# ALVI-Labs/frankenstein

Hardware: AMD Instinct MI355X
Metric: neural frames/sec (train fwd+bwd+AdamW, whole job) (higher is better)
Workload: dtype bf16; 1 GPU; brainformer-small (6L d=384 6x64 heads, N=6144 tokens) + 2-block perceiver, L1 head; fwd+bwd+clip+AdamW; per_gpu_batch=32, global_batch=32, frames_T=600, electrodes=256, parallelism=dp1, weights=random-init (seed 42)

## Files before the change

frankenstein_amd/csrc/elementwise.hip:

```cpp
#include "fk_common.h"

namespace {

template <typename T>
__global__ void rope_kernel(T* x, int64_t B, int64_t T_, int64_t ld, int rot_cols, int D, const float* table,
                            int64_t table_bs, int64_t pos_off, float sgn) {
  constexpr int N = VecIO<T>::N;
  const int cpr = rot_cols / N;
  const int64_t total = B * T_ * cpr;
  for (int64_t i = blockIdx.x * (int64_t)blockDim.x + threadIdx.x; i < total; i += (int64_t)gridDim.x * blockDim.x) {
    const int ch = (int)(i % cpr);
    const int64_t row = i / cpr, t = row % T_, b = row / T_;
    const int col = ch * N, d = col % D;
    T* px = x + row * ld + col;
    const float* tb = table + b * table_bs + ((pos_off + t) * (D / 2) + d / 2) * 2;
    float v[N], o[N];
    VecIO<T>::load(px, v);
#pragma unroll
    for (int j = 0; j < N / 2; ++j) {
      const float c = tb[2 * j], s = sgn * tb[2 * j + 1];
      o[2 * j] = v[2 * j] * c - v[2 * j + 1] * s;
      o[2 * j + 1] = v[2 * j] * s + v[2 * j + 1] * c;
    }
    VecIO<T>::store(px, o);
// ... 35 lines not shown
}
template <typename T>
__global__ void swiglu_bwd_kernel(const T* h13, const T* dg, T* dh13, int64_t rows, int H) {
  constexpr int N = VecIO<T>::N;
  const int cpr = H / N;
  const int64_t total = rows * cpr;
  for (int64_t i = blockIdx.x * (int64_t)blockDim.x + threadIdx.x; i < total; i += (int64_t)gridDim.x * blockDim.x) {
    const int64_t r = i / cpr;
    const int c = (int)(i % cpr) * N;
    float a[N], b[N], d[N], oa[N], ob[N];
    VecIO<T>::load(h13 + r * 2 * H + c, a);
    VecIO<T>::load(h13 + r * 2 * H + H + c, b);
    VecIO<T>::load(dg + r * H + c, d);
#pragma unroll
    for (int j = 0; j < N; ++j) {
      const float sg = sigmoidf_(a[j]);
      oa[j] = d[j] * b[j] * sg * (1.0f + a[j] * (1.0f - sg));
      ob[j] = d[j] * a[j] * sg;
    }
    VecIO<T>::store(dh13 + r * 2 * H + c, oa);
    VecIO<T>::store(dh13 + r * 2 * H + H + c, ob);
  }
}
template <typename T>
__global__ void gelu_fwd_kernel(const T* x, T* y, int64_t nvec) {
  constexpr int N = VecIO<T>::N;
  for (int64_t i = blockIdx.x * (int64_t)blockDim.x + threadIdx.x; i < nvec; i += (int64_t)gridDim.x * blockDim.x) {
    float a[N], o[N];
    VecIO<T>::load(x + i * N, a);
#pragma unroll
    for (int j = 0; j < N; ++j) o[j] = fk_gelu(a[j]);
    VecIO<T>::store(y + i * N, o);
  }
}
template <typename T>
__global__ void dropout_kernel(const T* x, const T* res, T* y, int64_t nvec, const unsigned* seed, unsigned site, unsigned thresh, float ks) {
  constexpr int N = VecIO<T>::N;
  const DropKey key = drop_key(seed, site, thresh);
  for (int64_t i = blockIdx.x * (int64_t)blockDim.x + threadIdx.x; i < nvec; i += (int64_t)gridDim.x * blockDim.x) {
    float a[N], o[N];
    VecIO<T>::load(x + i * N, a);
    if (res) VecIO<T>::load(res + i * N, o);
    const int64_t e0 = i * N;
    const unsigned row = drop_row(key, (unsigned)(e0 >> 32));
#pragma unroll
    for (int j = 0; j < N; ++j) {
      const float v = drop_keep(key, row, (unsigned)e0 + j) ? a[j] * ks : 0.0f;
      o[j] = res ? o[j] + v : v;
    }
    VecIO<T>::store(y + i * N, o);
  }
}
template <typename T>
__global__ void gelu_bwd_kernel(const T* x, const T* dy, T* dx, int64_t nvec) {
  constexpr int N = VecIO<T>::N;
  for (int64_t i = blockIdx.x * (int64_t)blockDim.x + threadIdx.x; i < nvec; i += (int64_t)gridDim.x * blockDim.x) {
    float a[N], d[N], o[N];
    VecIO<T>::load(x + i * N, a);
    VecIO<T>::load(dy + i * N, d);
#pragma unroll
    for (int j = 0; j < N; ++j) {
      const float cdf = 0.5f * (1.0f + erff(a[j] * 0.70710678118654752f));
      const float pdf = 0.3989422804014327f * __expf(-0.5f * a[j] * a[j]);
      o[j] = d[j] * (cdf + a[j] * pdf);
    }
    VecIO<T>::store(dx + i * N, o);
  }
}

template <typename T>
__global__ void cast_pack_kernel(const float* src, int64_t lds, T* dst, int64_t ldd, int rows, int cols, int transpose,
                                 int rblk, int rstride, int roff) {
  const int64_t total = (int64_t)rows * cols;
  for (int64_t i = blockIdx.x * (int64_t)blockDim.x + threadIdx.x; i < total; i += (int64_t)gridDim.x * blockDim.x) {
    int r, c;
    if (transpose) { r = (int)(i % rows); c = (int)(i / rows); }
    else { r = (int)(i / cols); c = (int)(i % cols); }
    const int rd = rblk > 0 ? (r / rblk) * rstride + (r % rblk) + roff : r;
    const float v = src[(int64_t)r * lds + c];
    if (transpose) dst[(int64_t)c * ldd + rd] = from_f32<T>(v);
    else dst[(int64_t)rd * ldd + c] = from_f32<T>(v);
  }
}
template <typename T>
__global__ __launch_bounds__(256) void cast_pack_multi_kernel(const fk_pack_job* jobs, int njobs, int64_t total_chunks) {
  __shared__ float tile[32][33];
  for (int64_t ch = blockIdx.x; ch < total_chunks; ch += gridDim.x) {
    int lo = 0, hi = njobs - 1;
    while (lo < hi) {
      const int mid = (lo + hi + 1) >> 1;
      if (jobs[mid].chunk_begin <= ch) lo = mid; else hi = mid - 1;
    }
    const fk_pack_job jb = jobs[lo];
    T* dst = (T*)jb.dst;
    const int64_t local = ch - jb.chunk_begin;
    if (!jb.transpose) {
      const int64_t total = (int64_t)jb.rows * jb.cols, base = local * 1024;
#pragma unroll
      for (int q = 0; q < 4; ++q) {
        const int64_t i = base + q * 256 + threadIdx.x;
        if (i >= total) break;
        const int r = (int)(i / jb.cols), c = (int)(i % jb.cols);
        const int rd = jb.rblk > 0 ? (r / jb.rblk) * jb.rstride + (r % jb.rblk) + jb.roff : r;
        dst[(int64_t)rd * jb.ldd + c] = from_f32<T>(jb.src[(int64_t)r * jb.lds + c]);
      }
    } else {
      const int tcols = (jb.cols + 31) / 32;
      const int r0 = (int)(local / tcols) * 32, c0 = (int)(local % tcols) * 32;
      const int tx = threadIdx.x & 31, ty = threadIdx.x >> 5;
      __syncthreads();
#pragma unroll
      for (int q = 0; q < 4; ++q) {
        const int r = r0 + ty + 8 * q, c = c0 + tx;
        tile[ty + 8 * q][tx] = (r < jb.rows && c < jb.cols) ? jb.src[(int64_t)r * jb.lds + c] : 0.0f;
      }
      __syncthreads();
#pragma unroll
      for (int q = 0; q < 4; ++q) {
        const int c = c0 + ty + 8 * q, r = r0 + tx;
        if (r < jb.rows && c < jb.cols) {
          const int rd = jb.rblk > 0 ? (r / jb.rblk) * jb.rstride + (r % jb.rblk) + jb.roff : r;
          dst[(int64_t)c * jb.ldd + rd] = from_f32<T>(tile[tx][ty + 8 * q]);
        }
      }
    }
  }
}
template <typename TS, typename TD>
__global__ void cast_kernel(const TS* src, TD* dst, int64_t n) {
  for (int64_t i = blockIdx.x * (int64_t)blockDim.x + threadIdx.x; i < n; i += (int64_t)gridDim.x * blockDim.x)
    dst[i] = from_f32<TD>(to_f32<TS>(src[i]));
}
template <typename T>
__global__ void add_kernel(const T* a, const T* b, T* y, int64_t n) {
  for (int64_t i = blockIdx.x * (int64_t)blockDim.x + threadIdx.x; i < n; i += (int64_t)gridDim.x * blockDim.x)
    y[i] = from_f32<T>(to_f32<T>(a[i]) + to_f32<T>(b[i]));
}
template <typename T>
__global__ void copy2d_kernel(const T* src, int64_t lds, T* dst, int64_t ldd, int64_t rows, int64_t cols) {
  const int64_t total = rows * cols;
  for (int64_t i = blockIdx.x * (int64_t)blockDim.x + threadIdx.x; i < total; i += (int64_t)gridDim.x * blockDim.x)
    dst[(i / cols) * ldd + (i % cols)] = src[(i / cols) * lds + (i % cols)];
}

__global__ void add2d_kernel(const float* src, int64_t lds, float* dst, int64_t ldd, int64_t rows, int64_t cols) {
  const int64_t total = rows * cols;
  for (int64_t i = blockIdx.x * (int64_t)blockDim.x + threadIdx.x; i < total; i += (int64_t)gridDim.x * blockDim.x)
    dst[(i / cols) * ldd + (i % cols)] += src[(i / cols) * lds + (i % cols)];
}

template <typename T>
__global__ void gpt_embed_kernel(const int64_t* idx, const T* prefix, const float* wte, const float* wpe, T* out, int B,
                                 int t_ctx, int t_words, int dim, int vocab) {
  const int t_full = t_ctx + t_words;
  const int64_t total = (int64_t)B * t_full * dim;
  for (int64_t i = blockIdx.x * (int64_t)blockDim.x + threadIdx.x; i < total; i += (int64_t)gridDim.x * blockDim.x) {
    const int c = (int)(i % dim);
    const int64_t row = i / dim;
    const int t = (int)(row % t_full), b = (int)(row / t_full);
    float v;
    if (t < t_ctx) v = to_f32<T>(prefix[((int64_t)b * t_ctx + t) * dim + c]);
    else {
      int64_t id = idx[(int64_t)b * t_words + (t - t_ctx)];
      id = id < 0 ? 0 : (id >= vocab ? vocab - 1 : id);
      v = wte[id * dim + c];
    }
    out[i] = from_f32<T>(v + wpe[(int64_t)t * dim + c]);
  }
}
template <typename T>
__global__ void embed_bwd_kernel(const int64_t* idx, const T* dout, int64_t ldo_rows_per_b, int t_ctx, int t_words,
                                 float* dtable, int B, int dim, int vocab) {
  const int64_t total = (int64_t)B * t_words * dim;
  for (int64_t i = blockIdx.x * (int64_t)blockDim.x + threadIdx.x; i < total; i += (int64_t)gridDim.x * blockDim.x) {
    const int c = (int)(i % dim);
    const int64_t r = i / dim;
    const int j = (int)(r % t_words), b = (int)(r / t_words);
    int64_t id = idx[r];
    id = id < 0 ? 0 : (id >= vocab ? vocab - 1 : id);
    const float g = to_f32<T>(dout[((int64_t)b * ldo_rows_per_b + t_ctx + j) * dim + c]);
    atomicAdd(dtable + id * dim + c, g);
  }
}

template <typename TS, typename TD>
__global__ void gather_rows_kernel(const TS* src, int64_t src_bs, const int64_t* idx, int64_t idx_mod, TD* dst, int B, int n,
                                   int W, int scatter, int64_t dst_bs) {
  const int64_t total = (int64_t)B * n * W;
  for (int64_t i = blockIdx.x * (int64_t)blockDim.x + threadIdx.x; i < total; i += (int64_t)gridDim.x * blockDim.x) {
    const int c = (int)(i % W);
    const int64_t r = i / W;
    const int b = (int)(r / n), k = (int)(r % n);
    int64_t j = idx[r];
    if (idx_mod > 0) j %= idx_mod;
    if (scatter) dst[(int64_t)b * dst_bs + j * W + c] = from_f32<TD>(to_f32<TS>(src[(int64_t)b * src_bs + (int64_t)k * W + c]));
    else dst[(int64_t)b * dst_bs + (int64_t)k * W + c] = from_f32<TD>(to_f32<TS>(src[(int64_t)b * src_bs + j * W + c]));
  }
}
template <typename TS, typename TD>
__global__ __launch_bounds__(256) void gather_rows_vec_kernel(const TS* src, int64_t src_bs, const int64_t* idx, int64_t idx_mod, TD* dst, int B, int n,
                                                              int W, int scatter, int64_t dst_bs) {
  const int cpr = W >> 3;
  const int lane = threadIdx.x & 63;
  const int rpw = cpr >= 64 ? 1 : 64 / cpr;
  const int sub = cpr >= 64 ? 0 : lane / cpr;
// ... 310 lines not shown
```

frankenstein_amd/csrc/fk_common.h:

```cpp
#pragma once
#include <hip/hip_runtime.h>
#include <stdint.h>

#include "../../include/franken_hip.h"

typedef __bf16 bf16_t;
typedef __bf16 bf16x8 __attribute__((ext_vector_type(8)));
typedef __bf16 bf16x4 __attribute__((ext_vector_type(4)));
typedef __bf16 bf16x2 __attribute__((ext_vector_type(2)));
typedef float f32x16 __attribute__((ext_vector_type(16)));
typedef float f32x4 __attribute__((ext_vector_type(4)));
typedef float f32x2 __attribute__((ext_vector_type(2)));
typedef short s16x4 __attribute__((ext_vector_type(4)));
typedef unsigned int u32x4 __attribute__((ext_vector_type(4)));

#define FK_DEV __device__ __forceinline__

int fk_set_error(int code, const char* fmt, ...);
#define FK_CHECK_ARG(cond, ...)                                   \
  do {                                                            \
    if (!(cond)) return fk_set_error(FK_EINVAL, __VA_ARGS__);     \
  } while (0)
#define FK_CHECK_LAUNCH(name)                                                         \
  do {                                                                                \
    hipError_t e__ = hipGetLastError();                                               \
    if (e__ != hipSuccess) return fk_set_error(FK_ELAUNCH, "%s: %s", name, hipGetErrorString(e__)); \
  } while (0)

#define FK_DT_CHECK(name) FK_CHECK_ARG(dtype == FK_F32 || dtype == FK_BF16, name ": bad dtype %d", dtype)

static inline int64_t fk_cdiv(int64_t a, int64_t b) { return (a + b - 1) / b; }

constexpr int FK_TPB = 256;
static inline unsigned fk_grid(int64_t work, int64_t cap) {
  int64_t b = fk_cdiv(work, FK_TPB);
  if (b > cap) b = cap;
  if (b < 1) b = 1;
  return (unsigned)b;
}

#define FK_BY_DTYPE(dtype, T, ...)                                \
  do {                                                            \
    if ((dtype) == FK_BF16) { using T = bf16_t; __VA_ARGS__; }    \
    else { using T = float; __VA_ARGS__; }                        \
  } while (0)
#define FK_BY_DTYPE2(dtype_a, TA, dtype_b, TB, ...) FK_BY_DTYPE(dtype_a, TA, FK_BY_DTYPE(dtype_b, TB, __VA_ARGS__))

template <auto Kernel, typename Args>
static inline void fk_launch_lds(dim3 grid, dim3 block, size_t lds, hipStream_t s, const Args& a) {
  static const bool once = hipFuncSetAttribute(reinterpret_cast<const void*>(Kernel), hipFuncAttributeMaxDynamicSharedMemorySize, (int)lds) == hipSuccess;
  (void)once;
  hipLaunchKernelGGL(Kernel, grid, block, lds, s, a);
}

template <typename T> FK_DEV float to_f32(T v);
template <> FK_DEV float to_f32<float>(float v) { return v; }
template <> FK_DEV float to_f32<bf16_t>(bf16_t v) { return (float)v; }
template <typename T> FK_DEV T from_f32(float v);
template <> FK_DEV float from_f32<float>(float v) { return v; }
template <> FK_DEV bf16_t from_f32<bf16_t>(float v) { return (bf16_t)v; }

template <typename T> struct Frag;
template <> struct Frag<bf16_t> { bf16x8 v; };
template <> struct Frag<float> { float v[8]; };

template <typename T> FK_DEV void frag_zero(Frag<T>& f);
template <> FK_DEV void frag_zero<bf16_t>(Frag<bf16_t>& f) {
#pragma unroll
  for (int e = 0; e < 8; ++e) f.v[e] = (bf16_t)0.0f;
}
template <> FK_DEV void frag_zero<float>(Frag<float>& f) {
#pragma unroll
  for (int e = 0; e < 8; ++e) f.v[e] = 0.0f;
}

template <typename T> FK_DEV void frag_set(Frag<T>& f, int e, float x);
template <> FK_DEV void frag_set<bf16_t>(Frag<bf16_t>& f, int e, float x) { f.v[e] = (bf16_t)x; }
template <> FK_DEV void frag_set<float>(Frag<float>& f, int e, float x) { f.v[e] = x; }

template <typename T> FK_DEV void mma32(f32x16& acc, const Frag<T>& a, const Frag<T>& b);
template <> FK_DEV void mma32<bf16_t>(f32x16& acc, const Frag<bf16_t>& a, const Frag<bf16_t>& b) {
  acc = __builtin_amdgcn_mfma_f32_32x32x16_bf16(a.v, b.v, acc, 0, 0, 0);
}
template <> FK_DEV void mma32<float>(f32x16& acc, const Frag<float>& a, const Frag<float>& b) {
#pragma unroll
// ... 4 lines not shown
FK_DEV int acc_row_of_slot(int s, int h, int e) { return 16 * s + 8 * (e >> 2) + 4 * h + (e & 3); }

template <typename T> FK_DEV void frag_from_acc(Frag<T>& f, const f32x16& x, int s) {
#pragma unroll
  for (int e = 0; e < 8; ++e) frag_set<T>(f, e, x[8 * s + e]);
}

template <typename T> FK_DEV void frag_load_contig(Frag<T>& f, const T* p);
template <> FK_DEV void frag_load_contig<bf16_t>(Frag<bf16_t>& f, const bf16_t* p) {
  f.v = *reinterpret_cast<const bf16x8*>(p);
}
template <> FK_DEV void frag_load_contig<float>(Frag<float>& f, const float* p) {
  f32x4 a = *reinterpret_cast<const f32x4*>(p);
  f32x4 b = *reinterpret_cast<const f32x4*>(p + 4);
#pragma unroll
  for (int e = 0; e < 4; ++e) { f.v[e] = a[e]; f.v[4 + e] = b[e]; }
}

FK_DEV bf16x4 lds_read_tr4(const bf16_t* p) {
  s16x4 r = __builtin_amdgcn_ds_read_tr16_b64_v4i16(
      (__attribute__((address_space(3))) s16x4*)(__attribute__((address_space(3))) void*)p);
  return __builtin_bit_cast(bf16x4, r);
}

FK_DEV float fk_gelu(float x) { return 0.5f * x * (1.0f + erff(x * 0.70710678118654752f)); }

template <int STOP = 1> FK_DEV float wave_sum(float v) {
#pragma unroll
  for (int o = 32; o >= STOP; o >>= 1) v += __shfl_xor(v, o, 64);
  return v;
}
template <int STOP = 1> FK_DEV float wave_max(float v) {
#pragma unroll
  for (int o = 32; o >= STOP; o >>= 1) v = fmaxf(v, __shfl_xor(v, o, 64));
  return v;
}

FK_DEV unsigned fk_mix32(unsigned x) {
  x ^= x >> 16; x *= 0x7feb352du; x ^= x >> 15; x *= 0x846ca68bu; x ^= x >> 16;
  return x;
}
struct DropKey { unsigned seed, salt, thresh; };
FK_DEV DropKey drop_key(const unsigned* seed_ptr, unsigned site, unsigned thresh) {
  return DropKey{seed_ptr[0], seed_ptr[1] * 0x85EBCA6Bu + site, thresh};
}
FK_DEV unsigned drop_row(const DropKey& k, unsigned hi) { return fk_mix32(fk_mix32(hi ^ k.seed) + k.salt); }
FK_DEV bool drop_keep(const DropKey& k, unsigned row, unsigned lo) { return fk_mix32(row ^ (lo * 0x9E3779B9u)) >= k.thresh; }

template <bool NT, typename V> FK_DEV void fk_st(V* q, const V& v) {
  if constexpr (NT) __builtin_nontemporal_store(v, q);
  else *q = v;
}

template <typename T, bool NT = false> struct VecIO;
template <bool NT> struct VecIO<bf16_t, NT> {
  static constexpr int N = 8;
  FK_DEV static void load(const bf16_t* p, float (&v)[8]) {
    bf16x8 a = *reinterpret_cast<const bf16x8*>(p);
#pragma unroll
    for (int i = 0; i < 8; ++i) v[i] = (float)a[i];
  }
  FK_DEV static void store(bf16_t* p, const float (&v)[8]) {
    bf16x8 a;
#pragma unroll
    for (int i = 0; i < 8; ++i) a[i] = (bf16_t)v[i];
    fk_st<NT>(reinterpret_cast<bf16x8*>(p), a);
  }
};
template <bool NT> struct VecIO<float, NT> {
  static constexpr int N = 4;
  FK_DEV static void load(const float* p, float (&v)[4]) {
    f32x4 a = *reinterpret_cast<const f32x4*>(p);
#pragma unroll
    for (int i = 0; i < 4; ++i) v[i] = a[i];
  }
  FK_DEV static void store(float* p, const float (&v)[4]) {
    f32x4 a;
#pragma unroll
    for (int i = 0; i < 4; ++i) a[i] = v[i];
    *reinterpret_cast<f32x4*>(p) = a;
  }
};

FK_DEV unsigned xcd_remap(unsigned bid, unsigned nwg) {
  const unsigned q = nwg >> 3, r = nwg & 7u, x = bid & 7u, i = bid >> 3;
  return (x < r ? x * (q + 1) : r * (q + 1) + (x - r) * q) + i;
}
```

frankenstein_amd/csrc/gemm.hip:

```cpp
#include <type_traits>

#include "fk_common.h"

namespace {

#ifndef FK_EPI_UNROLL
#define FK_EPI_UNROLL 1
#endif
#include "gemm_tile.h"

struct NtArgs {
  const void* A; const void* B; void* C;
  const void* bias; const void* res;
  int64_t lda, ldb, ldc, ldr, res_rows;
  int M, N, K, vec_epi;
  int mode;
  void* aux; int64_t ldaux;
  const float* rope_table; int64_t rope_bs; int rope_T, rope_off, rope_D, rope_cols;
  int rope_qcols; int64_t rope_qoff;
};

#ifndef FK_NT_STORES_GEMM
#define FK_NT_STORES_GEMM 1
#endif
// ... 1213 lines not shown
#endif
      __builtin_amdgcn_sched_barrier(0);
    }
  };
  using Yes = std::true_type;
  using No = std::false_type;
  using Vm0 = std::integral_constant<int, 0>;
  using Vm1 = std::integral_constant<int, PER>;
#pragma unroll
  for (int s = 0; s < TG_NS - 1; ++s)
    if (s < nk)
#pragma unroll
      for (int j = 0; j < PER; ++j) piece(s, j);
  if (nk > 0) {
    if (nk >= 3) vm_wait_barrier<2 * PER>(); else if (nk == 2) vm_wait_barrier<PER>(); else vm_wait_barrier<0>();
#pragma unroll
    for (int q = 0; q < NF; ++q) frag(f0, S0{}, q, 0);
#ifdef FK_TN_PROBE_HOIST
#pragma unroll
    for (int q = 0; q < NF; ++q) frag(f1, S1{}, q, 0);
#endif
    int kt = 0;
    for (; kt + TG_NS - 1 < nk; ++kt) step(Yes{}, Yes{}, Vm1{});
    if (kt + 2 < nk) { step(Yes{}, No{}, Vm1{}); ++kt; }
    if (kt + 1 < nk) step(Yes{}, No{}, Vm0{});
    step(No{}, No{}, Vm0{});
  }

  float* out = (p.nsplit > 1) ? p.ws + (int64_t)split * p.N1 * p.N2 : p.C;
  const int64_t ldo = (p.nsplit > 1) ? p.N2 : p.ldc;
  const bool accum = (p.nsplit == 1) && p.accumulate;
#pragma unroll
  for (int j = 0; j < NJ; ++j) {
    const int n = b0 + wn * WB + j * 32 + li;
#pragma unroll
    for (int i = 0; i < 3; ++i)
#pragma unroll
      for (int r = 0; r < 16; ++r) {
        const int m = a0 + wm * 96 + i * 32 + acc_row(r, lh);
        float* dst = out + (int64_t)m * ldo + n;
        *dst = accum ? (*dst + acc[i][j][r]) : acc[i][j][r];
      }
  }
}

template <bool IL>
__global__ __launch_bounds__(256) void reduce_slabs4_kernel(const float* ws, float* C, float* C1, int64_t ldc, int N1, int N2, int nsplit, int accumulate) {
  const int64_t total = (int64_t)N1 * N2, total4 = total >> 2;
  const int n2v = N2 >> 2;
  for (int64_t i = blockIdx.x * (int64_t)blockDim.x + threadIdx.x; i < total4; i += (int64_t)gridDim.x * blockDim.x) {
    const f32x4* src = reinterpret_cast<const f32x4*>(ws) + i;
    f32x4 s = {0.0f, 0.0f, 0.0f, 0.0f};
    int k = 0;
    for (; k + 8 <= nsplit; k += 8) {
      f32x4 v[8];
#pragma unroll
      for (int u = 0; u < 8; ++u) v[u] = src[(int64_t)(k + u) * total4];
#pragma unroll
      for (int u = 0; u < 8; ++u) s += v[u];
    }
    for (; k < nsplit; ++k) s += src[(int64_t)k * total4];
    int64_t r = i / n2v;
    float* base = C;
    if constexpr (IL) {
      if (r & 4) base = C1;
      r = (r >> 3) * 4 + (r & 3);
    }
    f32x4* dst = reinterpret_cast<f32x4*>(base + r * ldc + (i % n2v) * 4);
    if (accumulate) s += *dst;
    *dst = s;
  }
}
__global__ void reduce_slabs_kernel(const float* ws, float* C, int64_t ldc, int N1, int N2, int nsplit, int accumulate) {
  const int64_t total = (int64_t)N1 * N2;
  for (int64_t i = blockIdx.x * (int64_t)blockDim.x + threadIdx.x; i < total; i += (int64_t)gridDim.x * blockDim.x) {
    float s = 0.0f;
    for (int k = 0; k < nsplit; ++k) s += ws[k * total + i];
    float* dst = C + (i / N2) * ldc + (i % N2);
    *dst = accumulate ? (*dst + s) : s;
  }
}

template <typename T>
__global__ __launch_bounds__(256) void colsum_partial_kernel(const T* X, int64_t ld, float* part, int rows, int cols, int rows_per_blk) {
  constexpr int N = 16 / sizeof(T);
  __shared__ float red[256 * N];
  const int r0 = blockIdx.y * rows_per_blk, r1 = min(rows, r0 + rows_per_blk);
  const int cvt = (cols + N - 1) / N;
  {
    const int cv0 = blockIdx.x * 256;
    const int cvn = min(256, cvt - cv0), groups = 256 / cvn;
    const int vec = threadIdx.x % cvn, grp = threadIdx.x / cvn;
    float acc[N];
#pragma unroll
    for (int e = 0; e < N; ++e) acc[e] = 0.0f;
    if (grp < groups) {
      const T* p = X + (int64_t)(cv0 + vec) * N;
      for (int r = r0 + grp; r < r1; r += groups) {
        if constexpr (sizeof(T) == 2) {
          bf16x8 v = *reinterpret_cast<const bf16x8*>(p + (int64_t)r * ld);
#pragma unroll
          for (int e = 0; e < N; ++e) acc[e] += (float)v[e];
        } else {
          f32x4 v = *reinterpret_cast<const f32x4*>(p + (int64_t)r * ld);
#pragma unroll
          for (int e = 0; e < N; ++e) acc[e] += v[e];
        }
      }
    }
    __syncthreads();
#pragma unroll
    for (int e = 0; e < N; ++e) red[threadIdx.x * N + e] = acc[e];
    __syncthreads();
    if (threadIdx.x < cvn) {
#pragma unroll
      for (int e = 0; e < N; ++e) {
        float sm = 0.0f;
        for (int g2 = 0; g2 < groups; ++g2) sm += red[(g2 * cvn + threadIdx.x) * N + e];
        part[(int64_t)blockIdx.y * cols + (cv0 + threadIdx.x) * N + e] = sm;
      }
    }
  }
}
template <typename T>
__global__ void colsum_partial_scalar_kernel(const T* X, int64_t ld, float* part, int rows, int cols, int rows_per_blk) {
  const int c = blockIdx.x * blockDim.x + threadIdx.x;
  if (c >= cols) return;
  const int r0 = blockIdx.y * rows_per_blk, r1 = min(rows, r0 + rows_per_blk);
  float s = 0.0f;
  for (int r = r0; r < r1; ++r) s += to_f32<T>(X[(int64_t)r * ld + c]);
  part[(int64_t)blockIdx.y * cols + c] = s;
}
__global__ __launch_bounds__(256) void colsum_final_kernel(const float* part, float* out, int cols, int nblk, int accumulate) {
  __shared__ float red[256];
  const int c = blockIdx.x * 64 + (threadIdx.x & 63), g = threadIdx.x >> 6;
  float s = 0.0f;
  if (c < cols)
    for (int k = g; k < nblk; k += 4) s += part[(int64_t)k * cols + c];
  red[threadIdx.x] = s;
  __syncthreads();
  if (g == 0 && c < cols) {
    const float t = (red[threadIdx.x] + red[threadIdx.x + 64]) + (red[threadIdx.x + 128] + red[threadIdx.x + 192]);
    out[c] = accumulate ? out[c] + t : t;
  }
}

int tn_splits(int64_t M, int64_t N1, int64_t N2, int bkm) {
  const int64_t tiles = fk_cdiv(N1, BM) * fk_cdiv(N2, BN);
  int64_t want = fk_cdiv(1024, tiles);
  const int64_t maxs = fk_cdiv(M, (int64_t)bkm * 4);
  if (want >= 8) want = (want + 7) / 8 * 8;
  if (want > maxs) want = maxs;
  if (want < 1) want = 1;
  return (int)want;
}
bool tn_big_ok(int64_t M, int64_t N1, int64_t N2, int dtype) {
  return dtype == FK_BF16 && M % TG_K == 0 && M >= 16384 && N1 % TG_A == 0 && (N2 % TG_B == 0 || N2 % 192 == 0);
}
int tn_big_tb(int64_t N1, int64_t N2) {
  if (N2 % TG_B != 0) return 192;
  return (N2 % 192 == 0 && N1 >= 2048) ? 192 : TG_B;
}
int tn_big_splits(int64_t M, int64_t N1, int64_t N2) {
  const int64_t tiles = (N1 / TG_A) * (N2 / tn_big_tb(N1, N2));
  static const int mult = [] { const char* e = getenv("FK_TN_SPLIT_MULT"); const int v = e ? atoi(e) : 1; return v < 1 ? 1 : (v > 8 ? 8 : v); }();
  int64_t want = 256 / tiles * mult;
  const int64_t maxs = M / 512;
  if (want > maxs) want = maxs;
  if (want < 1) want = 1;
  return (int)want;
}
int colsum_blocks(int64_t rows) {
  int64_t b = fk_cdiv(rows, 256);
  if (b > 512) b = 512;
  if (b < 1) b = 1;
  return (int)b;
}

}

bool fk_qkv_rope_fused_ok(int64_t M, int64_t N, int64_t K, int64_t lda, int64_t ldb, int64_t ldc, bool has_bias, int64_t T, int64_t D, int64_t rot_cols, int64_t q_cols, int dtype);
int fk_qkv_rope_fused_launch(const void* A, int64_t lda, const void* W, int64_t ldb, void* C, int64_t ldc, int64_t M, int64_t N, const float* table, int64_t table_bs, int64_t T, int64_t pos_off, int64_t rot_cols, int64_t q_cols, int64_t q_off, void* stream);
bool fk_mlp_up_fused_ok(int64_t M, int64_t H, int64_t K, int64_t lda, int64_t ldb, int64_t ldh, int64_t ldg, int dtype);
int fk_mlp_up_fused_launch(const void* A, int64_t lda, const void* W13, int64_t ldb, void* H13, int64_t ldh, void* G, int64_t ldg, int64_t M, int64_t H, void* stream);

extern "C" {

struct RopeSpec { const float* table; int64_t bs; int T, off, D, cols; int qcols; int64_t qoff; };

static NtRoute nt_route(int64_t M, int64_t N, int64_t K, int dtype, bool vec_epi, int mode, bool has_rope) {
  const int64_t nwg = fk_cdiv(M, BM) * fk_cdiv(N, BN);
  const bool glds = dtype == FK_BF16 && (K % 64 == 0);
  const char* ring_min_env = getenv("FK_NT_RING_MIN_TILES");
  const int ring_min = ring_min_env ? atoi(ring_min_env) : 128;
  const bool wide = glds && M >= 4096 && vec_epi && fk_cdiv(M, 256) * fk_cdiv(N, 256) >= ring_min;
  if (wide && (N % 256 == 0 || (N % 128 == 0 && N >= 1024))) return NT_RING2;
  if (wide && N % 192 == 0 && N % 256 != 0 && N <= 768 && mode == 0 && !has_rope) return NT_RING192;
  if (wide && N % 128 == 0) return NT_RING128;
  if (glds && M >= 4096 && N % 256 == 0 && vec_epi) return NT_BIG;
  if (glds && nwg <= 256) return NT_GLDS4;
  return glds ? NT_GLDS : NT_STAGED;
}
// ... 117 lines not shown
  FK_CHECK_ARG(M > 0 && N1 > 0 && N2 > 0, "fk_gemm_tn_route: empty problem");
  return tn_plan(M, N1, N2, dtype, nsplit, rows_per_split);
}

size_t fk_gemm_tn_workspace_bytes(int64_t M, int64_t N1, int64_t N2, int dtype) {
  int ns;
  tn_plan(M, N1, N2, dtype, &ns, nullptr);
  return ns > 1 ? (size_t)ns * N1 * N2 * sizeof(float) : 0;
}

static int launch_tn(const void* A, int64_t lda, const void* B, int64_t ldb, float* C, float* C1, int64_t ldc, int64_t M, int64_t N1,
                     int64_t N2, int accumulate, int dtype, void* workspace, size_t workspace_bytes, void* stream) {
  FK_CHECK_ARG(dtype == FK_F32 || dtype == FK_BF16, "fk_gemm_tn: bad dtype %d", dtype);
  const int vec = dtype == FK_BF16 ? 8 : 4;
  FK_CHECK_ARG(M > 0 && N1 > 0 && N2 > 0, "fk_gemm_tn: empty problem");
  FK_CHECK_ARG(M < (1LL << 31) && N1 < (1LL << 31) && N2 < (1LL << 31), "fk_gemm_tn: dims must fit int32");
  FK_CHECK_ARG(N1 % vec == 0 && N2 % vec == 0 && lda % vec == 0 && ldb % vec == 0,
               "fk_gemm_tn: N1/N2/lda/ldb must be multiples of %d (N1=%lld N2=%lld)", vec, (long long)N1, (long long)N2);
  FK_CHECK_ARG(((uintptr_t)A & 15) == 0 && ((uintptr_t)B & 15) == 0, "fk_gemm_tn: A/B must be 16-byte aligned");
  int ns;
  int64_t rps;
  const int tb = tn_plan(M, N1, N2, dtype, &ns, &rps);
  const bool big = tb != 0;
  const size_t need = ns > 1 ? (size_t)ns * N1 * N2 * sizeof(float) : 0;
  FK_CHECK_ARG(workspace_bytes >= need && (need == 0 || workspace), "fk_gemm_tn: workspace too small (%zu < %zu)", workspace_bytes, need);
  if (C1)
    FK_CHECK_ARG(ns > 1 && N1 % 8 == 0 && N2 % 4 == 0 && ldc % 4 == 0 && (((uintptr_t)C | (uintptr_t)C1 | (uintptr_t)workspace) & 15) == 0,
                 "fk_gemm_tn_swiglu: needs a split plan (see fk_gemm_tn_route), N1 %% 8 == 0, N2 %% 4 == 0 and 16-byte aligned destinations");
  TnArgs p{A, B, C, (float*)workspace, lda, ldb, ldc, (int)M, (int)N1, (int)N2, (int)rps, ns, accumulate};
  dim3 grid((unsigned)(fk_cdiv(N1, BM) * fk_cdiv(N2, BN) * ns)), block(NTHREADS);
  hipStream_t s = (hipStream_t)stream;
  if (big) {
    dim3 bgrid((unsigned)((N1 / TG_A) * (N2 / tb) * ns));
    if (tb == 192) {
      constexpr int LDS192 = TG_NS * (TG_A_BYTES + TG_K * 512);
      fk_launch_lds<gemm_tn_big_kernel<192>>(bgrid, dim3(512), LDS192, s, p);
    } else {
      fk_launch_lds<gemm_tn_big_kernel<128>>(bgrid, dim3(512), TG_NS * TG_STAGE, s, p);
    }
  } else if (dtype == FK_BF16) hipLaunchKernelGGL((gemm_tn_kernel<bf16_t>), grid, block, 4 * TILE_BYTES, s, p);
  else hipLaunchKernelGGL((gemm_tn_kernel<float>), grid, block, 4 * TILE_BYTES, s, p);
  FK_CHECK_LAUNCH("fk_gemm_tn");
  if (ns > 1) {
    const int64_t total = N1 * N2;
    if (N2 % 4 == 0 && ldc % 4 == 0 && (((uintptr_t)C | (uintptr_t)workspace) & 15) == 0) {
      int nb = (int)fk_cdiv(total / 4, 256);
      if (nb > 2048) nb = 2048;
      if (C1) hipLaunchKernelGGL(reduce_slabs4_kernel<true>, dim3(nb), dim3(256), 0, s, (const float*)workspace, C, C1, ldc, (int)N1, (int)N2, ns, accumulate);
      else hipLaunchKernelGGL(reduce_slabs4_kernel<false>, dim3(nb), dim3(256), 0, s, (const float*)workspace, C, C1, ldc, (int)N1, (int)N2, ns, accumulate);
    } else {
      int nb = (int)fk_cdiv(total, 256);
      if (nb > 2048) nb = 2048;
      hipLaunchKernelGGL(reduce_slabs_kernel, dim3(nb), dim3(256), 0, s, (const float*)workspace, C, ldc, (int)N1, (int)N2, ns, accumulate);
    }
    FK_CHECK_LAUNCH("fk_gemm_tn(reduce)");
  }
  return FK_OK;
}

int fk_gemm_tn(const void* A, int64_t lda, const void* B, int64_t ldb, float* C, int64_t ldc, int64_t M, int64_t N1,
               int64_t N2, int accumulate, int dtype, void* workspace, size_t workspace_bytes, void* stream) {
  return launch_tn(A, lda, B, ldb, C, nullptr, ldc, M, N1, N2, accumulate, dtype, workspace, workspace_bytes, stream);
}

int fk_gemm_tn_swiglu(const void* A, int64_t lda, const void* B, int64_t ldb, float* d_up, float* d_gate, int64_t ldc, int64_t M,
                      int64_t H, int64_t N2, int dtype, void* workspace, size_t workspace_bytes, void* stream) {
  FK_CHECK_ARG(d_up && d_gate && H > 0 && H % 4 == 0, "fk_gemm_tn_swiglu: needs both destinations and H %% 4 == 0");
  return launch_tn(A, lda, B, ldb, d_up, d_gate, ldc, M, 2 * H, N2, 1, dtype, workspace, workspace_bytes, stream);
}

size_t fk_colsum_workspace_bytes(int64_t rows, int64_t cols) { return (size_t)colsum_blocks(rows) * cols * sizeof(float); }

int fk_colsum(const void* X, int64_t ld, float* out, int64_t rows, int64_t cols, int accumulate, int dtype,
              void* workspace, size_t workspace_bytes, void* stream) {
  FK_CHECK_ARG(dtype == FK_F32 || dtype == FK_BF16, "fk_colsum: bad dtype %d", dtype);
  FK_CHECK_ARG(rows > 0 && cols > 0 && rows < (1LL << 31) && cols < (1LL << 31), "fk_colsum: bad shape");
  const int nb = colsum_blocks(rows);
  FK_CHECK_ARG(workspace && workspace_bytes >= (size_t)nb * cols * sizeof(float), "fk_colsum: workspace too small");
  const int rpb = (int)fk_cdiv(rows, nb);
  hipStream_t s = (hipStream_t)stream;
  const int vec = dtype == FK_BF16 ? 8 : 4;
  if (cols % vec == 0 && ld % vec == 0 && ((uintptr_t)X & 15) == 0) {
    dim3 grid((unsigned)fk_cdiv(fk_cdiv(cols, vec), 256), (unsigned)nb), block(256);
    if (dtype == FK_BF16) hipLaunchKernelGGL(colsum_partial_kernel<bf16_t>, grid, block, 0, s, (const bf16_t*)X, ld, (float*)workspace, (int)rows, (int)cols, rpb);
    else hipLaunchKernelGGL(colsum_partial_kernel<float>, grid, block, 0, s, (const float*)X, ld, (float*)workspace, (int)rows, (int)cols, rpb);
  } else {
    dim3 grid((unsigned)fk_cdiv(cols, 256), (unsigned)nb), block(256);
    if (dtype == FK_BF16) hipLaunchKernelGGL(colsum_partial_scalar_kernel<bf16_t>, grid, block, 0, s, (const bf16_t*)X, ld, (float*)workspace, (int)rows, (int)cols, rpb);
    else hipLaunchKernelGGL(colsum_partial_scalar_kernel<float>, grid, block, 0, s, (const float*)X, ld, (float*)workspace, (int)rows, (int)cols, rpb);
  }
  FK_CHECK_LAUNCH("fk_colsum(partial)");
  hipLaunchKernelGGL(colsum_final_kernel, dim3((unsigned)fk_cdiv(cols, 64)), dim3(256), 0, s, (const float*)workspace, out, (int)cols, nb, accumulate);
  FK_CHECK_LAUNCH("fk_colsum(final)");
  return FK_OK;
}

}
```

Measured before the change: 401,200 frames/s.

## Fuse colsum final reduction via last-block counters and vectorize cast-pack kernel

The column-sum partial kernel now elects the last-finishing block per column tile through a per-stream atomic counter, and that block does the final cross-block reduction itself. This removes the separate colsum_final launch. The cast_pack_multi kernel now gives each block a contiguous range of chunks and advances the job index linearly instead of binary-searching per chunk. It also uses 4-wide vector loads and stores in both the plain and transposed paths. The counter scheme adds device-global state keyed by stream, and it relies on relaxed atomics plus fences being correct.

```diff
diff --git a/frankenstein_amd/csrc/elementwise.hip b/frankenstein_amd/csrc/elementwise.hip
--- a/frankenstein_amd/csrc/elementwise.hip
+++ b/frankenstein_amd/csrc/elementwise.hip
@@ -141,45 +141,77 @@
     else dst[(int64_t)rd * ldd + c] = from_f32<T>(v);
   }
 }
+template <typename T> FK_DEV void pack_store4(T* p, const float (&v)[4]) {
+  if constexpr (sizeof(T) == 2) {
+    bf16x4 o;
+#pragma unroll
+    for (int e = 0; e < 4; ++e) o[e] = (bf16_t)v[e];
+    *reinterpret_cast<bf16x4*>(p) = o;
+  } else {
+    *reinterpret_cast<f32x4*>(p) = f32x4{v[0], v[1], v[2], v[3]};
+  }
+}
+FK_DEV int pack_row(const fk_pack_job& jb, int r) { return jb.rblk > 0 ? (r / jb.rblk) * jb.rstride + (r % jb.rblk) + jb.roff : r; }
 template <typename T>
 __global__ __launch_bounds__(256) void cast_pack_multi_kernel(const fk_pack_job* jobs, int njobs, int64_t total_chunks) {
   __shared__ float tile[32][33];
-  for (int64_t ch = blockIdx.x; ch < total_chunks; ch += gridDim.x) {
-    int lo = 0, hi = njobs - 1;
-    while (lo < hi) {
-      const int mid = (lo + hi + 1) >> 1;
-      if (jobs[mid].chunk_begin <= ch) lo = mid; else hi = mid - 1;
-    }
+  const int64_t per = (total_chunks + gridDim.x - 1) / gridDim.x;
+  int64_t ch = blockIdx.x * per;
+  const int64_t end = min(total_chunks, ch + per);
+  if (ch >= end) return;
+  int lo = 0, hi = njobs - 1;
+  while (lo < hi) {
+    const int mid = (lo + hi + 1) >> 1;
+    if (jobs[mid].chunk_begin <= ch) lo = mid; else hi = mid - 1;
+  }
+  for (; ch < end; ++ch) {
+    while (lo + 1 < njobs && jobs[lo + 1].chunk_begin <= ch) ++lo;
     const fk_pack_job jb = jobs[lo];
     T* dst = (T*)jb.dst;
     const int64_t local = ch - jb.chunk_begin;
+    const bool src4 = jb.lds % 4 == 0 && ((uintptr_t)jb.src & 15) == 0;
+    const bool dst4 = jb.ldd % 4 == 0 && ((uintptr_t)jb.dst & (4 * sizeof(T) - 1)) == 0;
+    const bool rows4 = jb.rblk == 0 || (jb.rblk % 4 == 0 && jb.rstride % 4 == 0 && jb.roff % 4 == 0);
     if (!jb.transpose) {
-      const int64_t total = (int64_t)jb.rows * jb.cols, base = local * 1024;
-#pragma unroll
-      for (int q = 0; q < 4; ++q) {
-        const int64_t i = base + q * 256 + threadIdx.x;
-        if (i >= total) break;
-        const int r = (int)(i / jb.cols), c = (int)(i % jb.cols);
-        const int rd = jb.rblk > 0 ? (r / jb.rblk) * jb.rstride + (r % jb.rblk) + jb.roff : r;
-        dst[(int64_t)rd * jb.ldd + c] = from_f32<T>(jb.src[(int64_t)r * jb.lds + c]);
+      const int64_t total = (int64_t)jb.rows * jb.cols, i = local * 1024 + threadIdx.x * 4;
+      if (i >= total) continue;
+      const int r = (int)(i / jb.cols), c = (int)(i - (int64_t)r * jb.cols);
+      if (src4 && dst4 && jb.cols % 4 == 0) {
+        float v[4];
+        VecIO<float>::load(jb.src + (int64_t)r * jb.lds + c, v);
+        pack_store4<T>(dst + (int64_t)pack_row(jb, r) * jb.ldd + c, v);
+      } else {
+        int rr = r, cc = c;
+        for (int e = 0; e < 4 && i + e < total; ++e) {
+          dst[(int64_t)pack_row(jb, rr) * jb.ldd + cc] = from_f32<T>(jb.src[(int64_t)rr * jb.lds + cc]);
+          if (++cc == jb.cols) { cc = 0; ++rr; }
+        }
       }
     } else {
       const int tcols = (jb.cols + 31) / 32;
       const int r0 = (int)(local / tcols) * 32, c0 = (int)(local % tcols) * 32;
-      const int tx = threadIdx.x & 31, ty = threadIdx.x >> 5;
+      const int a = threadIdx.x >> 3, b4 = (threadIdx.x & 7) * 4;
       __syncthreads();
-#pragma unroll
-      for (int q = 0; q < 4; ++q) {
-        const int r = r0 + ty + 8 * q, c = c0 + tx;
-        tile[ty + 8 * q][tx] = (r < jb.rows && c < jb.cols) ? jb.src[(int64_t)r * jb.lds + c] : 0.0f;
+      {
+        const int r = r0 + a, c = c0 + b4;
+        float v[4] = {0.0f, 0.0f, 0.0f, 0.0f};
+        if (r < jb.rows) {
+          if (src4 && c + 3 < jb.cols) VecIO<float>::load(jb.src + (int64_t)r * jb.lds + c, v);
+          else
+            for (int e = 0; e < 4; ++e)
+              if (c + e < jb.cols) v[e] = jb.src[(int64_t)r * jb.lds + c + e];
+        }
+#pragma unroll
+        for (int e = 0; e < 4; ++e) tile[a][b4 + e] = v[e];
       }
       __syncthreads();
-#pragma unroll
-      for (int q = 0; q < 4; ++q) {
-        const int c = c0 + ty + 8 * q, r = r0 + tx;
-        if (r < jb.rows && c < jb.cols) {
-          const int rd = jb.rblk > 0 ? (r / jb.rblk) * jb.rstride + (r % jb.rblk) + jb.roff : r;
-          dst[(int64_t)c * jb.ldd + rd] = from_f32<T>(tile[tx][ty + 8 * q]);
+      const int c = c0 + a, r = r0 + b4;
+      if (c < jb.cols && r < jb.rows) {
+        if (dst4 && rows4 && r + 3 < jb.rows) {
+          const float v[4] = {tile[b4][a], tile[b4 + 1][a], tile[b4 + 2][a], tile[b4 + 3][a]};
+          pack_store4<T>(dst + (int64_t)c * jb.ldd + pack_row(jb, r), v);
+        } else {
+          for (int e = 0; e < 4 && r + e < jb.rows; ++e) dst[(int64_t)c * jb.ldd + pack_row(jb, r + e)] = from_f32<T>(tile[b4 + e][a]);
         }
       }
     }
diff --git a/frankenstein_amd/csrc/fk_common.h b/frankenstein_amd/csrc/fk_common.h
--- a/frankenstein_amd/csrc/fk_common.h
+++ b/frankenstein_amd/csrc/fk_common.h
@@ -1,6 +1,8 @@
 #pragma once
 #include <hip/hip_runtime.h>
 #include <stdint.h>
+
+#include <mutex>
 
 #include "../../include/franken_hip.h"
 
@@ -171,6 +173,39 @@
   }
 };
 
+constexpr int FK_RED_STREAMS = 64, FK_RED_PER_STREAM = 1024;
+namespace { __device__ unsigned fk_red_counters[FK_RED_STREAMS * FK_RED_PER_STREAM]; }
+
+static inline int fk_red_slot(hipStream_t s) {
+  static std::mutex mu;
+  static hipStream_t tab[FK_RED_STREAMS];
+  static int used = 0;
+  std::lock_guard<std::mutex> g(mu);
+  for (int i = 0; i < used; ++i)
+    if (tab[i] == s) return i * FK_RED_PER_STREAM;
+  if (used == FK_RED_STREAMS) return -1;
+  tab[used] = s;
+  return used++ * FK_RED_PER_STREAM;
+}
+
+FK_DEV void fk_red_store(float* p, float v) { __hip_atomic_store(p, v, __ATOMIC_RELAXED, __HIP_MEMORY_SCOPE_AGENT); }
+
+FK_DEV bool fk_red_last(unsigned* counter, unsigned n, unsigned* lds_word) {
+  asm volatile("s_waitcnt vmcnt(0)" ::: "memory");
+  __syncthreads();
+  if (threadIdx.x == 0) {
+    const bool last = __hip_atomic_fetch_add(counter, 1u, __ATOMIC_RELAXED, __HIP_MEMORY_SCOPE_AGENT) == n - 1;
+    if (last) {
+      __hip_atomic_store(counter, 0u, __ATOMIC_RELAXED, __HIP_MEMORY_SCOPE_AGENT);
+      __builtin_amdgcn_fence(__ATOMIC_ACQUIRE, "agent");
+      asm volatile("s_waitcnt vmcnt(0)" ::: "memory");
+    }
+    *lds_word = last ? 1u : 0u;
+  }
+  __syncthreads();
+  return *lds_word != 0u;
+}
+
 FK_DEV unsigned xcd_remap(unsigned bid, unsigned nwg) {
   const unsigned q = nwg >> 3, r = nwg & 7u, x = bid & 7u, i = bid >> 3;
   return (x < r ? x * (q + 1) : r * (q + 1) + (x - r) * q) + i;
diff --git a/frankenstein_amd/csrc/gemm.hip b/frankenstein_amd/csrc/gemm.hip
--- a/frankenstein_amd/csrc/gemm.hip
+++ b/frankenstein_amd/csrc/gemm.hip
@@ -1319,9 +1319,10 @@
 }
 
 template <typename T>
-__global__ __launch_bounds__(256) void colsum_partial_kernel(const T* X, int64_t ld, float* part, int rows, int cols, int rows_per_blk) {
+__global__ __launch_bounds__(256) void colsum_partial_kernel(const T* X, int64_t ld, float* part, int rows, int cols, int rows_per_blk,
+                                                              float* out, int accumulate, int slot) {
   constexpr int N = 16 / sizeof(T);
-  __shared__ float red[256 * N];
+  __shared__ __attribute__((aligned(16))) float red[256 * N];
   const int r0 = blockIdx.y * rows_per_blk, r1 = min(rows, r0 + rows_per_blk);
   const int cvt = (cols + N - 1) / N;
   {
@@ -1333,6 +1334,7 @@
     for (int e = 0; e < N; ++e) acc[e] = 0.0f;
     if (grp < groups) {
       const T* p = X + (int64_t)(cv0 + vec) * N;
+#pragma unroll 8
       for (int r = r0 + grp; r < r1; r += groups) {
         if constexpr (sizeof(T) == 2) {
           bf16x8 v = *reinterpret_cast<const bf16x8*>(p + (int64_t)r * ld);
@@ -1354,7 +1356,29 @@
       for (int e = 0; e < N; ++e) {
         float sm = 0.0f;
         for (int g2 = 0; g2 < groups; ++g2) sm += red[(g2 * cvn + threadIdx.x) * N + e];
-        part[(int64_t)blockIdx.y * cols + (cv0 + threadIdx.x) * N + e] = sm;
+        fk_red_store(part + (int64_t)blockIdx.y * cols + (cv0 + threadIdx.x) * N + e, sm);
+      }
+    }
+    if (slot < 0) return;
+    if (!fk_red_last(fk_red_counters + slot + blockIdx.x, gridDim.y, reinterpret_cast<unsigned*>(red))) return;
+    const int nblk = gridDim.y, g = threadIdx.x >> 6, v = threadIdx.x & 63;
+    const int cbeg = cv0 * N, cend = cbeg + cvn * N;
+    for (int c0 = cbeg; c0 < cend; c0 += 256) {
+      const int c = c0 + 4 * v;
+      f32x4 s = {0.0f, 0.0f, 0.0f, 0.0f};
+      if (c < cend) {
+#pragma unroll 16
+        for (int k = g; k < nblk; k += 4) s += *reinterpret_cast<const f32x4*>(part + (int64_t)k * cols + c);
+      }
+      __syncthreads();
+      *reinterpret_cast<f32x4*>(red + threadIdx.x * 4) = s;
+      __syncthreads();
+      if (g == 0 && c < cend) {
+#pragma unroll
+        for (int e = 0; e < 4; ++e) {
+          const float t = (red[4 * v + e] + red[256 + 4 * v + e]) + (red[512 + 4 * v + e] + red[768 + 4 * v + e]);
+          out[c + e] = accumulate ? out[c + e] + t : t;
+        }
       }
     }
   }
@@ -1638,8 +1662,13 @@
   const int vec = dtype == FK_BF16 ? 8 : 4;
   if (cols % vec == 0 && ld % vec == 0 && ((uintptr_t)X & 15) == 0) {
     dim3 grid((unsigned)fk_cdiv(fk_cdiv(cols, vec), 256), (unsigned)nb), block(256);
-    if (dtype == FK_BF16) hipLaunchKernelGGL(colsum_partial_kernel<bf16_t>, grid, block, 0, s, (const bf16_t*)X, ld, (float*)workspace, (int)rows, (int)cols, rpb);
-    else hipLaunchKernelGGL(colsum_partial_kernel<float>, grid, block, 0, s, (const float*)X, ld, (float*)workspace, (int)rows, (int)cols, rpb);
+    const int slot = (grid.x <= (unsigned)FK_RED_PER_STREAM && ((uintptr_t)workspace & 15) == 0) ? fk_red_slot(s) : -1;
+    if (dtype == FK_BF16) hipLaunchKernelGGL(colsum_partial_kernel<bf16_t>, grid, block, 0, s, (const bf16_t*)X, ld, (float*)workspace, (int)rows, (int)cols, rpb, out, accumulate, slot);
+    else hipLaunchKernelGGL(colsum_partial_kernel<float>, grid, block, 0, s, (const float*)X, ld, (float*)workspace, (int)rows, (int)cols, rpb, out, accumulate, slot);
+    if (slot >= 0) {
+      FK_CHECK_LAUNCH("fk_colsum");
+      return FK_OK;
+    }
   } else {
     dim3 grid((unsigned)fk_cdiv(cols, 256), (unsigned)nb), block(256);
     if (dtype == FK_BF16) hipLaunchKernelGGL(colsum_partial_scalar_kernel<bf16_t>, grid, block, 0, s, (const bf16_t*)X, ld, (float*)workspace, (int)rows, (int)cols, rpb);
```

New measurement: 402,500 frames/s (median of 6 runs). No clear change (+0.3%).
